# kaist-ina/stellatrain

Hardware: AMD Instinct MI355X
Metric: grad-codec GB/s (dense fp32 in) per GPU; thresholdv16 k=1% on 64 MiB bucket (higher is better)
Workload: dtype f32; 1 GPU; thresholdv16 k=167772 (1%) on 64 MiB fp32 buckets; step = 64 keys (4096 MiB) per GPU in 16 batched calls of 4, call j on stream j % 4; n=16777216, dst_len=167772, streams=4, parallelism=bucket-sharded x1, no collective

## Files before the change

include/stg/codec.h:

```cpp
#ifndef STG_CODEC_H
#define STG_CODEC_H

#include <stddef.h>
#include <stdint.h>

#ifdef __cplusplus
extern "C" {
#endif

#define STG_OK 0
#define STG_ERR_INVALID (-1)
#define STG_ERR_UNKNOWN (-2)
#define STG_ERR_HIP (-3)
#define STG_ERR_UNSUPPORTED (-4)
#define STG_ERR_DEVICE (-5)

typedef struct stg_codec *stg_codec_t;
typedef struct stg_sgd *stg_sgd_t;
typedef struct stg_adam *stg_adam_t;

int stg_codec_create(const char *method, int device, stg_codec_t *out);
int stg_codec_destroy(stg_codec_t h);
const char *stg_codec_name(stg_codec_t h);

// ... 21 lines not shown
int stg_codec_compress_batch_device(stg_codec_t h, const stg_bucket_t *buckets, size_t nbuckets, void *stream);

int stg_merge_compress_batch_device(stg_codec_t h, const stg_bucket_t *buckets, float *const *d_residuals,
                                    size_t nbuckets, void *stream);

int stg_merge_gather_compress_device(stg_codec_t h, const stg_bucket_t *bucket, float *d_residual,
                                     const float *const *d_grads, int num_gpus, void *stream);

int stg_codec_compress_wire_batch_device(stg_codec_t h, const stg_bucket_t *buckets, const int *flags,
                                         size_t nbuckets, void *stream);

typedef struct stg_send_task {
    stg_bucket_t bucket;
    float *d_residual;
    const float *const *d_grads;
    int num_gpus;
    int wire_flag;
} stg_send_task_t;

int stg_merge_send_batch_device(stg_codec_t h, const stg_send_task_t *tasks, size_t ntasks, void *stream);

int stg_codec_get_state(stg_codec_t h, const char *key, const void *key_ptr, float *threshold,
                        float *threshold_inc, void *stream);

int stg_codec_set_timing(stg_codec_t h, int enable);
int stg_codec_get_timing(stg_codec_t h, double *ms3, uint64_t *calls);

int stg_codec_debug_words(stg_codec_t h, void *stream, uint32_t *out, int n);

int stg_debug_tv16_scan_grid(int num_cu, int streams, int hw_queues, uint32_t chunks);

int stg_codec_check(stg_codec_t h);

int stg_scatter_merge_device(const uint32_t *d_idx, const float *d_val, size_t per_rank, int world, size_t n,
                             float *d_dense, uint8_t *d_mark, uint32_t *d_out_idx, float *d_out_val,
                             uint32_t *d_out_count, void *stream);
int stg_scatter_merge_check(void *stream);
int stg_scatter_merge_release(void *stream);

int stg_error_feedback_device(float *d_grad, size_t n, const uint32_t *d_idx, size_t numel, float *d_residual,
                              void *stream);

int stg_sgd_create(int device, float lr, float momentum, float dampening, float weight_decay, int nesterov,
                   int maximize, stg_sgd_t *out);
int stg_sgd_destroy(stg_sgd_t o);
int stg_sgd_optimize_raw_device(stg_sgd_t o, const char *name, float *d_param, uint32_t param_len,
// ... 106 lines not shown
```

stellatrain_amd/csrc/capi.cpp:

```cpp
#include <cmath>
#include <hip/hip_runtime.h>

#include <algorithm>
#include <array>
#include <map>
#include <cstdio>
#include <cstdlib>
#include <cstring>
#include <memory>
#include <mutex>
#include <string>
#include <unordered_map>
#include <vector>

#include <dlfcn.h>

#include "../../include/stg/codec.h"
#include "batch_pack.h"
#include "devbuf.h"
#include "scan_grid.h"
#include "ws.h"

namespace {

// ... 59 lines not shown
    stg::DevBuf<uint32_t> h_idx, h_count;
    uint32_t *pinned_count = nullptr;
    std::mutex wire_mu;
    stg::DevBuf<uint32_t> wst_pos;
    stg::DevBuf<float> wst_val;

    ~Workspace() {
        (void)hipSetDevice(device);
        if (stream) (void)hipStreamSynchronize(stream);
        if (pinned_count) (void)hipHostFree(pinned_count);
    }

    int init() {
        size_t off = 0;
        auto carve = [&](size_t bytes) {
            const size_t o = off;
            off = (off + bytes + 255) & ~size_t(255);
            return o;
        };
        const size_t o_ctl = carve(sizeof(stg::FillCtl));
        const size_t o_cp = carve(sizeof(stg::CallParams));
        const size_t o_rs = carve(sizeof(stg::RSel));
        const size_t o_fail = carve(sizeof(uint32_t));
        const size_t o_cand = carve(sizeof(uint32_t) * stg::CAND_WORDS * stg::MAX_BATCH);
        const size_t o_misc = carve(sizeof(uint32_t) * 64);
        const size_t o_tvt = carve(sizeof(uint64_t));
        const size_t o_wh = carve(sizeof(uint32_t) * 2 * stg::LNBIN);
        const size_t o_larr = carve(sizeof(uint32_t) * stg::LARR_WORDS);
        const size_t o_we = carve(sizeof(uint2) * stg::LNBIN * stg::LBCAP);
        const size_t o_crew = carve(sizeof(stg::CrewCtl) * stg::MAX_BATCH);
        const size_t o_tkc = carve(sizeof(stg::TopkCtl) * 2);
        const size_t o_tkf = carve(sizeof(uint32_t) * 2 * stg::TK2_FINE);
        HIP_TRY(fixed.reserve(off, stream, true));
        char *b = fixed.get();
        d.ctl = reinterpret_cast<stg::FillCtl *>(b + o_ctl);
        d.cp = reinterpret_cast<stg::CallParams *>(b + o_cp);
        d.rsel = reinterpret_cast<stg::RSel *>(b + o_rs);
        d.fail = reinterpret_cast<uint32_t *>(b + o_fail);
        d.cand = reinterpret_cast<uint32_t *>(b + o_cand);
        d.misc = reinterpret_cast<uint32_t *>(b + o_misc);
        d.tv_ticket = reinterpret_cast<uint64_t *>(b + o_tvt);
        d.whist = reinterpret_cast<uint32_t *>(b + o_wh);
        d.larr = reinterpret_cast<uint32_t *>(b + o_larr);
        d.went = reinterpret_cast<uint2 *>(b + o_we);
        d.crew = reinterpret_cast<stg::CrewCtl *>(b + o_crew);
        d.tkctl = reinterpret_cast<stg::TopkCtl *>(b + o_tkc);
        d.tkfine = reinterpret_cast<uint32_t *>(b + o_tkf);
// ... 802 lines not shown
        snprintf(b, sizeof b, "device failure flags 0x%x (details: stg_codec_check)", ws->pinned_count[1]);
        return fail(STG_ERR_DEVICE, b);
    }
    *out_count = *ws->pinned_count;
    return STG_OK;
}

int stg_codec_get_state(stg_codec_t h, const char *key, const void *key_ptr, float *threshold, float *threshold_inc,
                        void *stream) {
    if (!h) return fail(STG_ERR_INVALID, "null codec handle");
    HIP_TRY(hipSetDevice(h->device));
    KeyState *st = nullptr;
    {
        std::lock_guard<std::mutex> g(h->mu);
        auto it = h->slot_of.find(state_key(h->method, key, key_ptr));
        if (it == h->slot_of.end()) return fail(STG_ERR_INVALID, "key has no state yet");
        st = h->slot_ptr(it->second);
    }
    HIP_TRY(hipStreamSynchronize(static_cast<hipStream_t>(stream)));
    KeyState hs;
    HIP_TRY(hipMemcpy(&hs, st, sizeof hs, hipMemcpyDeviceToHost));
    if (threshold) *threshold = hs.t;
    if (threshold_inc) *threshold_inc = hs.inc;
    return STG_OK;
}

int stg_codec_set_timing(stg_codec_t h, int enable) {
    if (!h) return fail(STG_ERR_INVALID, "null codec handle");
    std::lock_guard<std::mutex> g(h->mu);
    h->timing = enable != 0;
    return STG_OK;
}

int stg_codec_get_timing(stg_codec_t h, double *ms3, uint64_t *calls) {
    if (!h || !ms3 || !calls) return fail(STG_ERR_INVALID, "null argument");
    HIP_TRY(hipSetDevice(h->device));
    std::lock_guard<std::mutex> g(h->mu);
    for (auto &e : h->ev_pending) {
        HIP_TRY(hipEventSynchronize(e[2]));
        float a = 0, b = 0, c = 0;
        HIP_TRY(hipEventElapsedTime(&a, e[0], e[1]));
        HIP_TRY(hipEventElapsedTime(&b, e[1], e[2]));
        HIP_TRY(hipEventElapsedTime(&c, e[0], e[2]));
        h->ms_acc[0] += a;
        h->ms_acc[1] += b;
        h->ms_acc[2] += c;
// ... 936 lines not shown
```

stellatrain_amd/csrc/common.h:

```cpp
#pragma once

#include <hip/hip_runtime.h>
#include <stdint.h>

#define STG_WG 256
#define STG_WAVES (STG_WG / 64)

struct KeyState {
    float t;
    float inc;
    uint32_t init;
    uint32_t pad;
};

enum : uint32_t {
    FAIL_SPIN_TIMEOUT = 1u,
    FAIL_CAND_OVERFLOW = 2u,
    FAIL_LEVELS = 4u,
    FAIL_SELECT = 8u,
};

namespace stg {

__device__ __forceinline__ uint32_t f2u(float f) { return __float_as_uint(f); }
__device__ __forceinline__ float u2f(uint32_t u) { return __uint_as_float(u); }

__device__ __forceinline__ uint32_t ford(float f) {
    const uint32_t u = __float_as_uint(f);
    return (u & 0x80000000u) ? ~u : (u | 0x80000000u);
}

template <int CTRL>
__device__ __forceinline__ float dpp_f(float v) {
    return __int_as_float(__builtin_amdgcn_mov_dpp(__float_as_int(v), CTRL, 0xF, 0xF, false));
}
// ... 149 lines not shown
```

stellatrain_amd/csrc/tv16.hip:

```cpp
#include <algorithm>
#include <cstdlib>

#include "scan_grid.h"
#include "tv16_dev.h"

namespace stg {

namespace {

using namespace tv16;
constexpr uint32_t kEfAux = 2;

constexpr uint32_t kTv16Ns = 11;
constexpr uint32_t FWG = (kTv16Ns + 1) * 64;
constexpr uint32_t FNW = FWG / 64;
constexpr uint32_t NS = kTv16Ns;
constexpr uint32_t FIN = NS;
static_assert(NS + 1 <= FNW && FWG <= 1024, "streaming group + finisher fit the workgroup");
constexpr uint32_t kTv16Nbuf = 5;
constexpr uint32_t kTv16ScanD = 3;
constexpr uint32_t NBUF = kTv16Nbuf;
constexpr uint32_t CIDR = 2 * NBUF;
constexpr uint32_t kTv16StageB = 72;
constexpr uint32_t kTv16WlB = 64;
// ... 50 lines not shown
    BucketDesc bk[MAX_BATCH];
    uint32_t nbk;
    uint32_t epoch;
    uint32_t K;
    FillCtl *ctl;
    ChunkDesc *desc;
    uint32_t *cand;
    uint32_t *fail;
    uint32_t *dbg;
};
constexpr uint32_t DBG_DEAD = 1, DBG_DEAD_MAX = 2, DBG_LAUNCHES = 4;
constexpr uint32_t CC_DEAD = 16;

struct Lds {
    float4 stage[NBUF][STAGE_B * 4];
    uint32_t stage_line[NBUF][STAGE_B];
    uint64_t wl[NBUF][WL_B];
    uint32_t nst[NBUF];
    uint32_t nwl[NBUF];
    uint32_t qcnt[NBUF];
    uint32_t wcnt[NBUF];
    uint32_t sdone[NBUF];
    float tval[NBUF], incv[NBUF];
    uint32_t cid[CIDR];
    uint32_t cok[CIDR];
    uint32_t mid[CIDR];
    uint32_t fdone;
    uint4 gb[GB];
};
static_assert(sizeof(Lds) <= TV16_SCAN_LDS, "two scan workgroups and a fill workgroup share a CU");

__device__ __forceinline__ constexpr uint32_t spin_site(uint32_t site) { return FAIL_SPIN_TIMEOUT | (1u << (8 + site)); }

struct Ctx {
    const BatchArgs &A;
    Lds &L;
    uint32_t G, w;
    FillCtl *ctlp;
    uint32_t *candp;
    uint32_t *failp;

    __device__ __forceinline__ uint32_t tag(uint32_t kind) const { return (A.epoch << 8) | kind; }
    __device__ __forceinline__ FillCtl *ctl() const { return ctlp; }
    __device__ __forceinline__ CallCtl *cc() const { return &ctlp->cc[A.epoch & 1u]; }
    __device__ __forceinline__ uint32_t *cand(uint32_t b) const { return candp + (size_t)b * CAND_WORDS; }
    __device__ __forceinline__ void fail(uint32_t bits) const { g_or(failp, bits); }
// ... 3 lines not shown
            st_sc1(failp + 2, w);
            st_sc1(failp + 3, x0);
            st_sc1(failp + 4, x1);
            st_sc1(failp + 5, x2);
            st_sc1(failp + 6, A.epoch);
        }
        uint32_t *rec = failp + 8 + 4 * site;
        if (atomicCAS(rec, 0u, w + 1u) == 0u) {
            st_sc1(rec + 1, x0);
            st_sc1(rec + 2, x1);
            st_sc1(rec + 3, x2);
        }
        for (uint32_t b = 0; b < A.nbk; ++b) st_sc1(A.bk[b].count_out, POISON_COUNT);
    }
    __device__ __forceinline__ uint32_t bucket_of(uint32_t k) const {
        uint32_t b = 0;
        while (b + 1 < A.nbk && k >= A.bk[b + 1].cs) ++b;
        return b;
    }
};

constexpr uint32_t TAG_AGG = 1, TAG_DEC = TV16_TAG_DEC;
constexpr uint32_t DEC_B = TV16_DEC_B, DEC_WIN = TV16_DEC_WIN, DEC_TAIL = TV16_DEC_TAIL;
constexpr uint32_t WIN = TV16_WIN;

template <int STAGE, bool EF, uint32_t SCAN_D>
__device__ __forceinline__ void scan_chunk(Ctx &C, uint32_t j, uint32_t k, uint32_t s) {
    Lds &L = C.L;
    const uint32_t par = j % NBUF;
    if (j >= NBUF) {
        uint64_t st2 = 0;
        uint32_t spins = 0;
        for (; lds_ld(&L.fdone) < j + 1 - NBUF; ++spins) {
            __builtin_amdgcn_s_sleep(2);
            if (spin_expired(spins, st2)) { if (flane() == 0) C.spin_fail(1, j, lds_ld(&L.fdone), s); break; }
        }
    }
    const uint32_t b = C.bucket_of(k);
    const BucketDesc &d = C.A.bk[b];
    const uint32_t c = k - d.cs;
    const uint32_t L0 = c * TV16_CHUNK;
    const uint32_t nl = d.nb > L0 ? std::min(TV16_CHUNK, d.nb - L0) : 0u;
    const float t = uni(d.state->t);
    const uint32_t lane = flane(), q = lane & 3;
    if (s == 0 && lane == 0) { L.tval[par] = t; L.incv[par] = uni(d.state->inc); }
    const uint32_t tb = f2u(t);
    const uint32_t wlo = tb > WIN ? tb - WIN : 0u;
    const uint32_t steps = (nl + 15) / 16;
    const uint32_t mine = steps > s ? (steps - s + NS - 1) / NS : 0u;
    uint32_t cnt_w = 0, win_w = 0;
    const __amdgpu_buffer_rsrc_t rsrc = __builtin_amdgcn_make_buffer_rsrc(
        const_cast<float *>(d.src + (size_t)L0 * 16), 0, nl * 64u, 0x00020000);
    const uint32_t lane_line = s * 16 + (lane >> 2);
    const __amdgpu_buffer_rsrc_t rsrc_r = __builtin_amdgcn_make_buffer_rsrc(
        EF ? d.resid + (size_t)L0 * 16 : nullptr, 0, (EF && d.resid) ? nl * 64u : 0u, 0x00020000);
    auto store_r = [&](uint32_t m, float4 x) {
        uint32_t voff = lane_line * 64u + q * 16u;
        asm volatile("" : "+v"(voff));
        u4v t4;
        t4.x = __float_as_uint(x.x); t4.y = __float_as_uint(x.y); t4.z = __float_as_uint(x.z); t4.w = __float_as_uint(x.w);
        __builtin_amdgcn_raw_buffer_store_b128(t4, rsrc_r, voff + m * (NS * 1024u), 0, kEfAux );
    };
    auto load = [&](uint32_t m) -> float4 {
        uint32_t voff = lane_line * 64u + q * 16u;
        asm volatile("" : "+v"(voff));
        const u4v t4 = __builtin_amdgcn_raw_buffer_load_b128(rsrc, voff + m * (NS * 1024u), 0, 2 );
        return make_float4(__uint_as_float(t4.x), __uint_as_float(t4.y), __uint_as_float(t4.z),
                           __uint_as_float(t4.w));
    };
    float4 v[SCAN_D];
// ... 136 lines not shown
}

template <int STAGE>
__device__ __forceinline__ void finish_chunk(Ctx &C, uint32_t j, uint32_t k) {
    Lds &L = C.L;
    const uint32_t par = j % NBUF;
    const uint32_t lane = flane();
    uint64_t st5 = 0;
    for (uint32_t spins = 0; lds_ld(&L.sdone[par]) < NS; ++spins) {
        __builtin_amdgcn_s_sleep(1);
        if (spin_expired(spins, st5)) { if (lane == 0) C.spin_fail(3, j, lds_ld(&L.sdone[par]), k); break; }
    }
    if (STAGE == 1 || STAGE == 3) {
        release(C, par, j);
        return;
    }
    const uint32_t b = C.bucket_of(k);
    const BucketDesc &d = C.A.bk[b];
    const uint32_t c = k - d.cs;
    const uint32_t L0 = c * TV16_CHUNK;
    const uint32_t nl = d.nb > L0 ? std::min(TV16_CHUNK, d.nb - L0) : 0u;
    const uint32_t qw = uni(L.qcnt[par]);
    const float t = uni(L.tval[par]), inc = uni(L.incv[par]);

    uint32_t P = 0, Wbef = 0;
    if (c) prefix_counts(C, b, c, P, Wbef);
    const uint32_t ww = uni(L.wcnt[par]);

    const uint32_t kb = d.dst_len / 16, r = d.dst_len % 16;
    const uint32_t lim = kb + (r ? 1u : 0u);
    const bool vec = aligned16(d);
    if (P < lim && qw) {
        if (qw <= STAGE_B) {
            const uint32_t q = lane & 3;
            for (uint32_t e0 = 0; e0 < qw; e0 += 16) {
                const uint32_t e = e0 + (lane >> 2);
                if (e >= qw) continue;
                const uint32_t i = L.stage_line[par][e];
                uint32_t g = P;
                for (uint32_t x = 0; x < qw; ++x) g += L.stage_line[par][x] < i;
                if (g >= lim) continue;
                const uint32_t pos = (L0 + i) * 16 + 4 * q;
                const uint32_t len = g == kb ? r : 16u;
                const uint32_t off = 16 * g + 4 * q;
                const float4 x = L.stage[par][e * 4 + q];
                const uint32_t bi = pos + (uint32_t)d.idx_offset;
// ... 19 lines not shown
                    const uint32_t g = base + (uint32_t)__popcll(m & below_mask(lane));
                    if (g < lim) emit_line(d, vec, (L0 + i) * 16, 16 * g, g == kb ? r : 16u);
                }
                base += (uint32_t)__popcll(m);
            }
        }
    }

    if (Wbef + ww + 1 <= CAND_CAP) {
        const uint32_t nwl = uni(lds_ld(&L.nwl[par]));
        uint32_t *cu = C.cand(b);
        uint32_t *cp = cu + CAND_CAP, *ci = cu + 2 * CAND_CAP;
        const uint32_t tb = f2u(t);
        if (nwl <= WL_B && qw <= STAGE_B) {
            static_assert(WL_B == 64, "one listed entry per lane");
            const uint64_t e = lane < nwl ? L.wl[par][lane] : ~0ull;
            const uint32_t mypos = (uint32_t)e;
            const uint32_t li = mypos / 16 - L0;
            uint32_t before = 0, qb = 0;
            for (uint32_t l = 0; l < nwl; ++l) before += (uint32_t)L.wl[par][l] < mypos;
            for (uint32_t x = 0; x < qw; ++x) qb += L.stage_line[par][x] < li;
            if (lane < nwl) {
                const uint32_t idx = Wbef + before;
                st_sc1(&cu[idx], (uint32_t)(e >> 32));
                st_sc1(&cp[idx], mypos);
                st_sc1(&ci[idx], L0 + li - P - qb);
            }
        } else {
            const uint32_t wlo = tb > WIN ? tb - WIN : 0u;
            uint32_t base = Wbef, qb = P;
            for (uint32_t i0 = 0; i0 < nl; i0 += 64) {
                const uint32_t i = i0 + lane;
                const float S = i < nl ? lane_line_sum(d.src + (size_t)(L0 + i) * 16) : 0.f;
                const uint32_t u = f2u(S);
                const bool qf = i < nl && S >= t;
                const bool wf = i < nl && u >= wlo && u < tb;
                const uint64_t mq = __ballot(qf), mw = __ballot(wf);
                if (wf) {
                    const uint32_t idx = base + (uint32_t)__popcll(mw & below_mask(lane));
                    st_sc1(&cu[idx], u);
                    st_sc1(&cp[idx], (L0 + i) * 16);
                    st_sc1(&ci[idx], L0 + i - (qb + (uint32_t)__popcll(mq & below_mask(lane))));
                }
                base += (uint32_t)__popcll(mw);
                qb += (uint32_t)__popcll(mq);
            }
        }
    }
    release(C, par, j);

    if (c + 1 == d.nc) {
        const uint32_t Qtot = P + qw, Wtot = Wbef + ww;
        const uint32_t c0 = Qtot >= lim ? d.dst_len : 16u * Qtot;
        bool tail_cand = false;
        float tail_key = 0.f;
        uint32_t ct = 0;
        if (c0 < d.dst_len && d.tl) {
            const float *tp = d.src + (size_t)d.nb * 16;
            float s = 0.f;
            for (uint32_t i = 0; i < d.tl; ++i) s += tp[i];
            s = uni(s);
            if (s * 16.0f >= t * (float)d.tl) ct = std::min(d.dst_len - c0, d.tl);
            else { tail_cand = true; tail_key = s * 16.0f / (float)d.tl; }
        }
        const uint32_t cnt = c0 + ct;
        const bool regimeB = cnt < d.dst_len;
        if (lane == 0) {
            if (ct) {
                const size_t p0 = (size_t)d.nb * 16;
                for (uint32_t i = 0; i < ct; ++i) {
                    put_pair(d, c0 + i, (uint32_t)(p0 + i) + (uint32_t)d.idx_offset, d.src[p0 + i]);
                }
            }
            d.state->t = regimeB ? (float)((double)t * 0.99) : t + inc;
            d.state->inc = inc;
            d.state->init = 1;
            st_sc1(d.count_out, (uint32_t)std::min<uint64_t>(d.dst_len, (uint64_t)d.nb * 16 + d.tl));
            if (ld_sc1(C.failp)) st_sc1(d.count_out, POISON_COUNT);
        }
        const uint32_t ncand = d.nb - Qtot;
        const uint32_t M = regimeB ? std::min((d.dst_len - cnt + 15u) / 16u, ncand) : 0u;
        uint32_t flags = 0;
        if (regimeB) flags = DEC_B | (tail_cand ? DEC_TAIL : 0u) | (Wtot >= M && Wtot + 1 <= CAND_CAP ? DEC_WIN : 0u);
        Decision &D = C.ctl()->dec[b];
        if (lane == 0) {
            st_sc1(&D.w[1], ((uint64_t)cnt << 32) | M);
            st_sc1(&D.w[2], ((uint64_t)Wtot << 32) | __float_as_uint(tail_key));
            st_sc1(&D.w[3], ((uint64_t)Qtot << 32) | __float_as_uint(t));
        }
        vm_drain();
        if (lane == 0) st_sc1(&D.w[0], ((uint64_t)C.tag(TAG_DEC) << 32) | flags);
    }
}

template <int STAGE, bool EF, bool LONE>
__global__ void __launch_bounds__(1024) __attribute__((amdgpu_waves_per_eu(LONE ? 6 : 8, 8)))
tv16_batch(BatchArgs A) {
    __shared__ Lds L;
    Ctx C{A, L, gridDim.x, blockIdx.x, A.ctl, A.cand, A.fail};
    {
        uint32_t *z = reinterpret_cast<uint32_t *>(&A.ctl->cc[(A.epoch + 1) & 1u]);
        constexpr uint32_t words = sizeof(CallCtl) / 4;
        const uint32_t per = (words + C.G - 1) / C.G;
        const uint32_t z0 = C.w * per, z1 = std::min(words, z0 + per);
        for (uint32_t i = z0 + threadIdx.x; i < z1; i += FWG) st_sc1(z + i, 0u);
    }
// ... 290 lines not shown
```

stellatrain_amd/csrc/tv16fill.hip:

```cpp
#ifndef STG_WIRE_EMIT
#define STG_WIRE_EMIT 0
#endif
#include <algorithm>
#include <cstddef>

#include "tv16_dev.h"

namespace stg {

namespace {

using namespace tv16;

constexpr uint32_t FILL_WG = 512;
constexpr uint32_t FNW_F = FILL_WG / 64;
constexpr uint32_t EMAX = 4096;
constexpr uint32_t VCAP = 6144;
constexpr uint32_t POS_LIM = (1u << 20) - 1;
constexpr uint32_t NONE = 0xffffffffu;
constexpr uint32_t NONE13 = 0x1fffu;
constexpr uint32_t CNONE = 0xffffffu;
constexpr uint32_t NBIN = 1024;
constexpr uint32_t NDEP = 20;
constexpr uint32_t PT = EMAX / FILL_WG;
constexpr uint32_t NJ = VCAP / FILL_WG;
constexpr uint32_t TCAP = 256;
constexpr uint32_t ECAP = 64;
static_assert(VCAP < NONE13, "13-bit node indices");
static_assert(NBIN << 8 == TV16_WIN, "output-sort bins of 256 ulps cover the window");

__device__ __forceinline__ uint32_t dkey_of_pos(uint32_t pos) {
    const uint32_t q = pos + 1, d = depth_of(q);
    return ((q << (19u - d)) << 5) | d;
}
__device__ __forceinline__ uint32_t dk_depth(uint32_t k) { return k & 31u; }
__device__ __forceinline__ uint32_t dk_pos(uint32_t k) { return ((k >> 5) >> (19u - (k & 31u))) - 1u; }
__device__ __forceinline__ uint32_t dk_anc(uint32_t k, uint32_t d) {
    return (((k >> 5) >> (19u - d)) << (19u - d) << 5) | d;
}
__device__ __forceinline__ uint32_t dk_left(uint32_t k) { return (k & ~31u) | (dk_depth(k) + 1); }
__device__ __forceinline__ uint32_t dk_right(uint32_t k) {
    return (((k >> 5) | (1u << (18u - dk_depth(k)))) << 5) | (dk_depth(k) + 1);
}
__device__ __forceinline__ int dk_lca(uint32_t a, uint32_t b) {
    const uint32_t m = min(dk_depth(a), dk_depth(b));
    const uint32_t x = ((a >> 5) ^ (b >> 5)) >> (19u - m);
    return x ? (int)m - (int)(32u - __clz(x)) : (int)m;
}

__device__ __forceinline__ uint32_t r_content(uint2 r) { return r.x & CNONE; }
__device__ __forceinline__ uint32_t r_pos(uint2 r) { return (r.x >> 24) | ((r.y & 0xfffu) << 8); }
__device__ __forceinline__ uint32_t r_right(uint2 r) { return (r.y >> 12) & NONE13; }
// ... 498 lines not shown
            } else {
                for (uint32_t c = 0; c < 4; ++c) {
                    if (4 * q + c < len) {
                        wire_put(oidx, oval, STG_WIRE_EMIT ? wflag : 0u, wend, o + c, bi + c, src[(size_t)pos + 4 * q + c]);
                    }
                }
            }
        }
        return;
    }
    constexpr uint32_t PRE = LONE ? 10 : 8, PREX = PRE;
    constexpr uint32_t KE = LONE ? 10 : 5;
    const uint32_t *cu = d.cand, *cl = d.cand + CAND_CAP, *ci = d.cand + 2 * CAND_CAP;
    uint32_t pk[PRE], pl[PREX], pc[PREX];
#pragma unroll
    for (uint32_t u = 0; u < PRE; ++u) {
        const uint32_t e = tid + u * FILL_WG;
        pk[u] = ld_sc1(&cu[e]);
        if (u < PREX) {
            pl[u] = ld_sc1(&cl[e]);
            pc[u] = ld_sc1(&ci[e]);
        }
    }
    static_assert(PRE * FILL_WG <= CAND_CAP, "prefetch inside the window buffer");
    const uint64_t w0 = ld_sc1(&D.w[0]), w1 = ld_sc1(&D.w[1]), w2 = ld_sc1(&D.w[2]), w3 = ld_sc1(&D.w[3]);
    const uint32_t failed = ld_sc1(A.fail);
    if ((uint32_t)(w0 >> 32) != ((A.epoch << 8) | TV16_TAG_DEC)) {
        if (tid == 0) { g_or(A.fail, FAIL_SPIN_TIMEOUT); st_sc1(d.count_out, POISON_COUNT); }
        return;
    }
    const uint32_t flags = (uint32_t)w0;
    if (!(flags & TV16_DEC_B) || failed) return;
    const uint32_t cnt = (uint32_t)(w1 >> 32), M = (uint32_t)w1;
    const uint32_t Wtot = (uint32_t)(w2 >> 32);
    const float tail_key = u2f((uint32_t)w2);
    const uint32_t Qtot = (uint32_t)(w3 >> 32);
    const float t = u2f((uint32_t)w3);
    const bool tail = (flags & TV16_DEC_TAIL) != 0;
    const uint32_t N = d.nb - Qtot + (tail ? 1u : 0u);
    const uint32_t rem = d.dst_len - cnt;
    if (!M && !tail) return;
    if (A.crew && crew_wants(flags, M, A.mode)) return;
    const uint32_t nhelp = LONE ? A.helpers : 0u;
    CallCtl *const ccp = A.cc;
    const uint32_t tb = f2u(t);
    const uint32_t wlo = tb > TV16_WIN ? tb - TV16_WIN : 0u;
    const bool tail_in = tail && tail_key >= u2f(wlo);
    bool fast = (flags & TV16_DEC_WIN) && N <= POS_LIM && Wtot + (tail_in ? 1u : 0u) > 0 && A.mode != 2u &&
                A.mode != 3u;
    if (!fast && tid == 0) {
        if (!(flags & TV16_DEC_WIN)) atomicAdd(&A.dbg[60], 1u);
        if (N > POS_LIM) atomicAdd(&A.dbg[61], 1u);
    }
    uint32_t *const key = S.u.a.key, *const cix = S.u.a.cix;
    auto kbin = [&](uint32_t kb) -> uint32_t {
        const float k = u2f(kb);
        if (k >= t) return 0u;
        if (!(k > 0.f)) return NBIN - 1;
        return min((tb - 1u - kb) >> 8, NBIN - 1);
    };
    auto okey = [&](uint32_t e) -> uint64_t { return (uint64_t)(~ford(u2f(key[e]))) << 32; };
    auto ksum = [&](uint32_t r) -> float { return u2f(key[S.ord[r]]); };
    uint32_t W = 0, Et = NONE;
    uint32_t *const lines_g = reinterpret_cast<uint32_t *>(d.heap);
    auto line_of = [&](uint32_t i) { return ld_sc1(&lines_g[S.ord[i]]); };
    auto line_lds = [&](uint32_t i) { return S.u.a.line[S.ord[i]]; };
    auto pops = [&](uint32_t &P, uint32_t &tail_rank) {
        for (uint32_t i = tid; i < W; i += FILL_WG)
            if (S.ord[i] == Et) S.flag = i;
        __syncthreads();
        tail_rank = S.flag;
        uint32_t npl = 0;
        for (uint32_t i = tid; i < W; i += FILL_WG) {
            const uint32_t off = 16u * i - (tail_rank < i ? 16u - d.tl : 0u);
            if (off < rem) npl = max(npl, i + 1);
        }
        npl = wave_max(npl);
        if ((tid & 63u) == 0) atomicMax(&S.npop, npl);
        __syncthreads();
        P = S.npop;
    };
    if (tid == 0) { S.flag = NONE; S.nv = 0; S.maxpos = 0; S.npop = 0; S.dmax = 0; S.rn = 0; S.nc = 0; S.nu = 0; S.et = NONE; }
    __syncthreads();
    uint32_t P0 = 0, tail_rank0 = NONE;
    if (fast) {
        SortScratch &X = S.u.a.s;
        stamp(0);
        for (uint32_t i = tid; i < NBIN; i += FILL_WG) X.bin[i] = 0;
        __syncthreads();
#pragma unroll
        for (uint32_t u = 0; u < PRE; ++u)
            if (tid + u * FILL_WG < Wtot) atomicAdd(&X.bin[kbin(pk[u])], 1u);
        for (uint32_t e = tid + PRE * FILL_WG; e < Wtot; e += FILL_WG) atomicAdd(&X.bin[kbin(ld_sc1(&cu[e]))], 1u);
        if (tail_in && tid == 0) atomicAdd(&X.bin[kbin(f2u(tail_key))], 1u);
        __syncthreads();
        stamp(0);
        {
            constexpr uint32_t PER = NBIN / FILL_WG;
            static_assert(PER == 2, "two bins per thread");
            const uint32_t c0 = X.bin[PER * tid], c1 = X.bin[PER * tid + 1], need = M + 2;
            uint32_t tot;
            const uint32_t run = blk_excl_scan<FNW_F>(c0 + c1, S.sh, &tot);
            X.bin[PER * tid] = X.cur[PER * tid] = run;
            X.bin[PER * tid + 1] = X.cur[PER * tid + 1] = run + c0;
            if (run < need && run + c0 >= need) { S.flag = PER * tid + 1; S.nv = run + c0; }
            else if (run + c0 < need && run + c0 + c1 >= need) { S.flag = PER * tid + 2; S.nv = run + c0 + c1; }
            if (tid == 0 && tot < need) { S.flag = NBIN; S.nv = tot; }
            __syncthreads();
        }
        const uint32_t cut = S.flag;
        W = S.nv;
        fast = W <= EMAX;
        if (!fast && tid == 0) atomicAdd(&A.dbg[62], 1u);
        if (fast) {
            auto keep = [&](uint32_t kb, uint32_t line, uint32_t cx, bool is_tail) {
                const uint32_t e = atomicAdd(&X.cur[kbin(kb)], 1u);
                key[e] = kb;
                S.u.a.line[e] = line;
                cix[e] = cx;
                st_sc1(&lines_g[e], line);
                if (is_tail) S.et = e;
            };
#pragma unroll
            for (uint32_t u = 0; u < PRE; ++u) {
                const uint32_t e = tid + u * FILL_WG;
                if (e >= Wtot || kbin(pk[u]) >= cut) continue;
                if (u < PREX) keep(pk[u], pl[u], pc[u], false);
                else keep(pk[u], ld_sc1(&cl[e]), ld_sc1(&ci[e]), false);
            }
            for (uint32_t e = tid + PRE * FILL_WG; e < Wtot; e += FILL_WG) {
                const uint32_t kb = ld_sc1(&cu[e]);
                if (kbin(kb) < cut) keep(kb, ld_sc1(&cl[e]), ld_sc1(&ci[e]), false);
            }
            if (tail_in && tid == 0 && kbin(f2u(tail_key)) < cut) keep(f2u(tail_key), d.nb * 16, N - 1, true);
            __syncthreads();
            stamp(0);
            for (uint32_t e = tid; e < W; e += FILL_WG) {
                const uint32_t bb = kbin(key[e]), lo = X.bin[bb], hi = X.cur[bb];
                const uint64_t k = okey(e) | cix[e];
                uint32_t r = lo;
                for (uint32_t x = lo; x < hi; ++x) r += (okey(x) | cix[x]) < k;
                S.ord[r] = (uint16_t)e;
            }
        }
        Et = S.et;
        __syncthreads();
        if (tid == 0) { S.flag = NONE; S.nv = 0; }
        __syncthreads();
    }
    if (fast) {
        stamp(0);
        pops(P0, tail_rank0);
        uint32_t tie_l = 0;
        for (uint32_t i = tid; i < P0; i += FILL_WG)
            if (i + 1 < W && ksum(i) == ksum(i + 1)) tie_l = 1;
        tie_l = wave_max(tie_l);
        if ((tid & 63u) == 0 && tie_l) S.nv = 1;
        __syncthreads();
        const bool ties = S.nv != 0;
        const uint32_t covered = 16u * W - (Et != NONE ? 16u - d.tl : 0u);
        fast = covered >= rem;
        if (!fast && tid == 0) atomicAdd(&A.dbg[63], 1u);
        if (fast && !ties) {
            emit_all<KE, LONE>(d, cnt, rem, P0, tail_rank0, line_lds, nhelp, ccp, order_g, ready_tag);
            count_path(0);
            stamp(5);
            return;
        }
    }
    if (fast) {
        const uint32_t pc = min(P0, W - 1);
        const float kc = ksum(pc);
        for (uint32_t r = tid; r < W; r += FILL_WG)
            if (ksum(r) == kc && (r + 1 == W || ksum(r + 1) != kc)) S.rn = r + 1;
        __syncthreads();
        fast = S.rn < EMAX;
    }
    if (fast) {
        const uint32_t Rn = S.rn;
        const uint32_t i0 = PT * tid;
        {
            uint32_t stm = 0, nsm = 0;
#pragma unroll
            for (uint32_t u = 0; u < PT; ++u) {
                const uint32_t r = i0 + u;
                if (r < Rn && (r == 0 || ksum(r - 1) != ksum(r))) { stm |= 1u << u; ++nsm; }
            }
            uint32_t tot;
// ... 53 lines not shown
                    }
                }
            }
            if ((__any(bad) || A.mode == 1u) && (tid & 63u) == 0) S.flag2 = 1;
            __syncthreads();
            stamp(0);
            if (!S.flag2) {
                uint16_t *const ord2 = S.u.a.s.tmp;
                for (uint32_t r = tid; r < Rn; r += FILL_WG) {
                    const uint32_t g = S.grp[r], kr = rf_key(cix[S.ord[r]]);
                    uint32_t o = g;
                    for (uint32_t x = g; x < Rn && S.grp[x] == g; ++x) o += rf_key(cix[S.ord[x]]) < kr;
                    ord2[o] = S.ord[r];
                }
                __syncthreads();
                for (uint32_t r = tid; r < Rn; r += FILL_WG) S.ord[r] = ord2[r];
                if (tid == 0) { S.flag = NONE; S.npop = 0; }
                __syncthreads();
                uint32_t P, tail_rank;
                pops(P, tail_rank);
                stamp(0);
                emit_all<KE, LONE>(d, cnt, rem, P, tail_rank, line_lds, nhelp, ccp, order_g, ready_tag);
                count_path(1);
                stamp(0);
                stamp(2);
                return;
            }
        }
        for (uint32_t r = tid; r < Rn; r += FILL_WG) S.u.b.dk[r] = dkey_of_pos(cix[S.ord[r]]);
        __syncthreads();
        counting_sort(S.u.b.s, S.u.b.eo, S.sh, Rn, [&](uint32_t r) { return S.u.b.dk[r] >> 15; },
                      [&](uint32_t r) { return (uint64_t)S.u.b.dk[r]; });
        stamp(0);
        uint32_t kq[PT + 1], rq[PT];
#pragma unroll
        for (uint32_t u = 0; u <= PT; ++u) kq[u] = i0 + u < Rn ? S.u.b.dk[S.u.b.eo[i0 + u]] : 0u;
#pragma unroll
        for (uint32_t u = 0; u < PT; ++u) rq[u] = i0 + u < Rn ? S.u.b.eo[i0 + u] : 0u;
        const uint32_t kp = (i0 >= 1 && i0 - 1 < Rn) ? S.u.b.dk[S.u.b.eo[i0 - 1]] : 0u;
        auto Lof = [&](uint32_t u) -> int {
            const uint32_t i = i0 + u;
            return (i >= 1 && i < Rn) ? dk_lca(u ? kq[u - 1] : kp, kq[u]) : -1;
        };
        uint32_t nmine = 0;
#pragma unroll
        for (uint32_t u = 0; u < PT; ++u) {
// ... 162 lines not shown
            nc = wave_sum(nc);
            if ((tid & 63u) == 0) { atomicMax(&S.maxpos, mp); atomicAdd(&S.nc, nc); }
            __syncthreads();
            fast = S.nc == Rn;
        }
        if (fast) {
            for (uint32_t r = tid; r < Rn; r += FILL_WG) {
                const uint32_t g = S.grp[r], kr = rf_key(S.u.f.fpos[r]);
                uint32_t o = g;
                for (uint32_t x = g; x < Rn && S.grp[x] == g; ++x) o += rf_key(S.u.f.fpos[x]) < kr;
                S.u.f.ord2[o] = S.ord[r];
            }
            __syncthreads();
            for (uint32_t r = tid; r < Rn; r += FILL_WG) S.ord[r] = S.u.f.ord2[r];
            if (tid == 0) { S.flag = NONE; S.npop = 0; }
            __syncthreads();
            uint32_t P, tail_rank;
            pops(P, tail_rank);
            stamp(0);
            if (STG_FILL_STAMPS && tid == 0 && b == 0) A.dbg[45] = P;
            if (S.maxpos + P < N && P <= Rn) {
                emit_all<KE, LONE>(d, cnt, rem, P, tail_rank, line_of, nhelp, ccp, order_g, ready_tag);
                count_path(2);
                stamp(1);
                return;
            }
            fast = false;
        }
    }
    __syncthreads();
    if ((flags & TV16_DEC_WIN) && A.mode != 2u) {
        const uint32_t P0 = (rem + 15u) / 16u, seln = min(P0 + 1u, N - 1u);
        if (Wtot >= seln + 1u || Wtot + (tail ? 1u : 0u) == N) {
            WideLds &Wl = *reinterpret_cast<WideLds *>(fill_lds);
            LeadIn I;
            I.lk = cu;
            I.lp = cl;
            I.lc = ci;
            I.n = Wtot;
            I.tail = tail ? 1u : 0u;
            I.tail_bits = f2u(tail_key);
            I.N = N;
            I.nb = d.nb;
            I.rem = rem;
            I.tl = d.tl;
            I.g = reinterpret_cast<uint32_t *>(d.heap);
            I.dbg = A.dbg;
            I.lvl1 = NONE;
            I.r1 = 0;
            I.gcap = 2u * (d.nb + 64u);
            I.positions = true;
            const LeadOut O = leader(Wl, I);
            if (O.ok) {
                const uint32_t *const opos = O.ordpos;
                emit_all<KE, LONE>(d, cnt, rem, O.P, O.tail_rank, [&](uint32_t i) { return ld_sc1(&opos[i]); }, nhelp,
                                   ccp, order_g, ready_tag);
                if (tid == 0) atomicAdd(&A.dbg[52], 1u);
                return;
            }
            if (tid == 0) atomicAdd(&A.dbg[54], 1u);
            __syncthreads();
        }
    }
    if (tid == 0) { S.flag = NONE; S.npop = 0; }
    __syncthreads();
    stamp(3);
    count_path(3);
    if (LONE && A.helpers && tid == 0) {
        st_sc1(&A.cc->pad[2], 0u);
        __builtin_amdgcn_s_waitcnt(0);
        st_sc1(&A.cc->pad[1], ready_tag);
    }
    full_path(S, d, cnt, N, t, tail, tail_key, A.fail);
    stamp(0);
}

}

constexpr size_t LFIN_LDS = std::max(std::max(sizeof(FillLds), sizeof(LfinLds)), sizeof(WideLdsBig));
static_assert(LFIN_LDS <= 160 * 1024, "one lfin workgroup per CU");
// ... 23 lines not shown
```

stellatrain_amd/csrc/ws.h:

```cpp
#pragma once

#include <hip/hip_runtime.h>
#include <stdint.h>

#include "common.h"

namespace stg {

constexpr uint32_t CAND_CAP = 8192;
constexpr uint32_t CAND_WORDS = 4 * CAND_CAP;
constexpr uint32_t TV16_WIN = 1u << 18;
constexpr uint32_t TV16_SCAN_LDS = 35584;

constexpr uint32_t TV_TILE = 8192;
constexpr uint32_t TOPK_SUP_CAP = 1024;
constexpr uint32_t TOPK_LIST_CAP = 4096;
constexpr uint32_t TOPK_LIST_TILES = 8192;
constexpr uint32_t TV_MAXG = 2048;
constexpr uint32_t TV_SCAP = 4096;

constexpr uint32_t RS_BINS = 2048;
constexpr uint32_t RS_SHARDS = 8;
constexpr uint32_t RS_SH_HIST = 4;

constexpr uint32_t MAX_BATCH = 32;
constexpr uint32_t TV16_CHUNK = 2048;
struct CallCtl {
    uint32_t next;
    uint32_t pad[31];
    uint32_t crew_ticket[32];
    uint32_t crew_done[32];
};
struct alignas(32) Decision {
    uint64_t w[4];
};
constexpr uint32_t TV16_DEC_B = 1, TV16_DEC_WIN = 2, TV16_DEC_TAIL = 4;
constexpr uint32_t TV16_TAG_DEC = 3;
constexpr uint32_t POISON_COUNT = 0xffffffffu;
struct FillCtl {
    CallCtl cc[2];
    Decision dec[MAX_BATCH];
};
struct alignas(16) ChunkDesc {
    uint64_t agg;
    uint64_t pad;
};

struct CallParams {
    float t;
    float inc;
    uint32_t pad[2];
};

struct RSel {
    uint32_t prefix;
    uint32_t mask;
    uint32_t rank;
    uint32_t cnt_gt;
    uint32_t done;
// ... 460 lines not shown
```

Baseline: 6189 GB/s.

## Adapt tv16 candidate window width per key and double candidate capacity

Replaces the fixed threshold-window width with a per-key adaptive width stored in the codec state. The width grows when the candidate list misses or overflows and shrinks after a run of calm calls. Candidate list capacity is doubled, writes beyond it are bounds-checked, and the fill's histogram bins scale with the window width. The aim is to keep more calls on the fast windowed fill path instead of falling back to the full path. The cost is a larger scratch carve, extra per-call state updates, and a deep-selection guard that can force some calls onto the slow path.

Result: no change. 6188 GB/s (-0.0%).

```diff
diff --git a/include/stg/codec.h b/include/stg/codec.h
--- a/include/stg/codec.h
+++ b/include/stg/codec.h
@@ -67,6 +67,8 @@
 
 int stg_codec_get_state(stg_codec_t h, const char *key, const void *key_ptr, float *threshold,
                         float *threshold_inc, void *stream);
+
+int stg_codec_get_window(stg_codec_t h, const char *key, uint32_t *width, uint32_t *calm, void *stream);
 
 int stg_codec_set_timing(stg_codec_t h, int enable);
 int stg_codec_get_timing(stg_codec_t h, double *ms3, uint64_t *calls);
diff --git a/stellatrain_amd/csrc/capi.cpp b/stellatrain_amd/csrc/capi.cpp
--- a/stellatrain_amd/csrc/capi.cpp
+++ b/stellatrain_amd/csrc/capi.cpp
@@ -105,7 +105,9 @@
         const size_t o_cp = carve(sizeof(stg::CallParams));
         const size_t o_rs = carve(sizeof(stg::RSel));
         const size_t o_fail = carve(sizeof(uint32_t));
-        const size_t o_cand = carve(sizeof(uint32_t) * stg::CAND_WORDS * stg::MAX_BATCH);
+        static_assert(stg::tv16win::cand_carve_words() >= (uint64_t)stg::CAND_WORDS * stg::MAX_BATCH,
+                      "the carve covers the lists of a full launch");
+        const size_t o_cand = carve(sizeof(uint32_t) * (size_t)stg::tv16win::cand_carve_words());
         const size_t o_misc = carve(sizeof(uint32_t) * 64);
         const size_t o_tvt = carve(sizeof(uint64_t));
         const size_t o_wh = carve(sizeof(uint32_t) * 2 * stg::LNBIN);
@@ -954,6 +956,24 @@
     HIP_TRY(hipMemcpy(&hs, st, sizeof hs, hipMemcpyDeviceToHost));
     if (threshold) *threshold = hs.t;
     if (threshold_inc) *threshold_inc = hs.inc;
+    return STG_OK;
+}
+
+int stg_codec_get_window(stg_codec_t h, const char *key, uint32_t *width, uint32_t *calm, void *stream) {
+    if (!h) return fail(STG_ERR_INVALID, "null codec handle");
+    HIP_TRY(hipSetDevice(h->device));
+    KeyState *st = nullptr;
+    {
+        std::lock_guard<std::mutex> g(h->mu);
+        auto it = h->slot_of.find(state_key(h->method, key, nullptr));
+        if (it == h->slot_of.end()) return fail(STG_ERR_INVALID, "key has no state yet");
+        st = h->slot_ptr(it->second);
+    }
+    HIP_TRY(hipStreamSynchronize(static_cast<hipStream_t>(stream)));
+    KeyState hs;
+    HIP_TRY(hipMemcpy(&hs, st, sizeof hs, hipMemcpyDeviceToHost));
+    if (width) *width = stg::tv16win::win_c(hs.win);
+    if (calm) *calm = stg::tv16win::win_calm(hs.win);
     return STG_OK;
 }
 
diff --git a/stellatrain_amd/csrc/common.h b/stellatrain_amd/csrc/common.h
--- a/stellatrain_amd/csrc/common.h
+++ b/stellatrain_amd/csrc/common.h
@@ -10,7 +10,7 @@
     float t;
     float inc;
     uint32_t init;
-    uint32_t pad;
+    uint32_t win;
 };
 
 enum : uint32_t {
diff --git a/stellatrain_amd/csrc/tv16.hip b/stellatrain_amd/csrc/tv16.hip
--- a/stellatrain_amd/csrc/tv16.hip
+++ b/stellatrain_amd/csrc/tv16.hip
@@ -96,6 +96,7 @@
     uint32_t wcnt[NBUF];
     uint32_t sdone[NBUF];
     float tval[NBUF], incv[NBUF];
+    uint32_t cwin[NBUF];
     uint32_t cid[CIDR];
     uint32_t cok[CIDR];
     uint32_t mid[CIDR];
@@ -145,7 +146,6 @@
 
 constexpr uint32_t TAG_AGG = 1, TAG_DEC = TV16_TAG_DEC;
 constexpr uint32_t DEC_B = TV16_DEC_B, DEC_WIN = TV16_DEC_WIN, DEC_TAIL = TV16_DEC_TAIL;
-constexpr uint32_t WIN = TV16_WIN;
 
 template <int STAGE, bool EF, uint32_t SCAN_D>
 __device__ __forceinline__ void scan_chunk(Ctx &C, uint32_t j, uint32_t k, uint32_t s) {
@@ -166,9 +166,10 @@
     const uint32_t nl = d.nb > L0 ? std::min(TV16_CHUNK, d.nb - L0) : 0u;
     const float t = uni(d.state->t);
     const uint32_t lane = flane(), q = lane & 3;
-    if (s == 0 && lane == 0) { L.tval[par] = t; L.incv[par] = uni(d.state->inc); }
+    const uint32_t cw = uni(d.state->win);
+    if (s == 0 && lane == 0) { L.tval[par] = t; L.incv[par] = uni(d.state->inc); L.cwin[par] = cw; }
     const uint32_t tb = f2u(t);
-    const uint32_t wlo = tb > WIN ? tb - WIN : 0u;
+    const uint32_t wlo = tv16win::win_lo(tb, tv16win::win_c(cw));
     const uint32_t steps = (nl + 15) / 16;
     const uint32_t mine = steps > s ? (steps - s + NS - 1) / NS : 0u;
     uint32_t cnt_w = 0, win_w = 0;
@@ -351,6 +352,7 @@
     const uint32_t nl = d.nb > L0 ? std::min(TV16_CHUNK, d.nb - L0) : 0u;
     const uint32_t qw = uni(L.qcnt[par]);
     const float t = uni(L.tval[par]), inc = uni(L.incv[par]);
+    const uint32_t cw = uni(L.cwin[par]), wc = tv16win::win_c(cw);
 
     uint32_t P = 0, Wbef = 0;
     if (c) prefix_counts(C, b, c, P, Wbef);
@@ -416,12 +418,16 @@
             for (uint32_t x = 0; x < qw; ++x) qb += L.stage_line[par][x] < li;
             if (lane < nwl) {
                 const uint32_t idx = Wbef + before;
-                st_sc1(&cu[idx], (uint32_t)(e >> 32));
-                st_sc1(&cp[idx], mypos);
-                st_sc1(&ci[idx], L0 + li - P - qb);
+                if (idx < CAND_CAP) {
+                    st_sc1(&cu[idx], (uint32_t)(e >> 32));
+                    st_sc1(&cp[idx], mypos);
+                    st_sc1(&ci[idx], L0 + li - P - qb);
+                } else {
+                    C.fail(FAIL_CAND_OVERFLOW);
+                }
             }
         } else {
-            const uint32_t wlo = tb > WIN ? tb - WIN : 0u;
+            const uint32_t wlo = tv16win::win_lo(tb, wc);
             uint32_t base = Wbef, qb = P;
             for (uint32_t i0 = 0; i0 < nl; i0 += 64) {
                 const uint32_t i = i0 + lane;
@@ -432,9 +438,13 @@
                 const uint64_t mq = __ballot(qf), mw = __ballot(wf);
                 if (wf) {
                     const uint32_t idx = base + (uint32_t)__popcll(mw & below_mask(lane));
-                    st_sc1(&cu[idx], u);
-                    st_sc1(&cp[idx], (L0 + i) * 16);
-                    st_sc1(&ci[idx], L0 + i - (qb + (uint32_t)__popcll(mq & below_mask(lane))));
+                    if (idx < CAND_CAP) {
+                        st_sc1(&cu[idx], u);
+                        st_sc1(&cp[idx], (L0 + i) * 16);
+                        st_sc1(&ci[idx], L0 + i - (qb + (uint32_t)__popcll(mq & below_mask(lane))));
+                    } else {
+                        C.fail(FAIL_CAND_OVERFLOW);
+                    }
                 }
                 base += (uint32_t)__popcll(mw);
                 qb += (uint32_t)__popcll(mq);
@@ -459,6 +469,8 @@
         }
         const uint32_t cnt = c0 + ct;
         const bool regimeB = cnt < d.dst_len;
+        const uint32_t ncand = d.nb - Qtot;
+        const uint32_t M = regimeB ? std::min((d.dst_len - cnt + 15u) / 16u, ncand) : 0u;
         if (lane == 0) {
             if (ct) {
                 const size_t p0 = (size_t)d.nb * 16;
@@ -469,13 +481,13 @@
             d.state->t = regimeB ? (float)((double)t * 0.99) : t + inc;
             d.state->inc = inc;
             d.state->init = 1;
+            d.state->win = tv16win::win_next(cw, regimeB, M, Wtot);
             st_sc1(d.count_out, (uint32_t)std::min<uint64_t>(d.dst_len, (uint64_t)d.nb * 16 + d.tl));
             if (ld_sc1(C.failp)) st_sc1(d.count_out, POISON_COUNT);
         }
-        const uint32_t ncand = d.nb - Qtot;
-        const uint32_t M = regimeB ? std::min((d.dst_len - cnt + 15u) / 16u, ncand) : 0u;
-        uint32_t flags = 0;
-        if (regimeB) flags = DEC_B | (tail_cand ? DEC_TAIL : 0u) | (Wtot >= M && Wtot + 1 <= CAND_CAP ? DEC_WIN : 0u);
+        uint32_t flags = wc << TV16_DEC_CSHIFT;
+        const bool holds = (Wtot >= M + 2u || Wtot == ncand) && Wtot >= M && tv16win::list_fits(Wtot);
+        if (regimeB) flags |= DEC_B | (tail_cand ? DEC_TAIL : 0u) | (holds ? DEC_WIN : 0u);
         Decision &D = C.ctl()->dec[b];
         if (lane == 0) {
             st_sc1(&D.w[1], ((uint64_t)cnt << 32) | M);
diff --git a/stellatrain_amd/csrc/tv16_window.h b/stellatrain_amd/csrc/tv16_window.h
--- /dev/null
+++ b/stellatrain_amd/csrc/tv16_window.h
@@ -0,0 +1,76 @@
+#pragma once
+
+#include <stdint.h>
+
+#if defined(__HIPCC__) || defined(__CUDACC__)
+#define TV16W_HD __host__ __device__
+#else
+#define TV16W_HD
+#endif
+
+namespace stg {
+namespace tv16win {
+
+constexpr uint32_t UNIT_LOG2 = 16;
+constexpr uint32_t C_BASE = 4;
+constexpr uint32_t C_MAX = 9;
+constexpr uint32_t CALM_CALLS = 32;
+constexpr uint32_t C_MASK = 0xffu, CALM_SHIFT = 8, CALM_MASK = 0xffu;
+static_assert(C_MAX <= C_MASK && CALM_CALLS <= CALM_MASK, "both fields fit their byte");
+static_assert(C_BASE >= 1 && C_BASE <= C_MAX, "the range is not empty");
+
+TV16W_HD constexpr uint32_t win_c(uint32_t word) {
+    return (word & C_MASK) < C_BASE ? C_BASE : (word & C_MASK) > C_MAX ? C_MAX : (word & C_MASK);
+}
+TV16W_HD constexpr uint32_t win_calm(uint32_t word) { return (word >> CALM_SHIFT) & CALM_MASK; }
+TV16W_HD constexpr uint32_t win_word(uint32_t c, uint32_t calm) { return (calm << CALM_SHIFT) | c; }
+TV16W_HD constexpr uint32_t win_ulps(uint32_t c) { return c << UNIT_LOG2; }
+TV16W_HD constexpr uint32_t win_lo(uint32_t tb, uint32_t c) { return tb > win_ulps(c) ? tb - win_ulps(c) : 0u; }
+
+constexpr uint32_t NBIN = 1024;
+constexpr uint32_t BIN_LOG2 = 8;
+static_assert((NBIN << BIN_LOG2) == win_ulps(C_BASE), "at the base width the bins are 256 ulps, as the one-bucket path's");
+TV16W_HD constexpr uint32_t bin_shift(uint32_t c) {
+    uint32_t s = 0;
+    while (((NBIN << BIN_LOG2) << s) < win_ulps(c)) ++s;
+    return s;
+}
+TV16W_HD constexpr uint32_t win_bin(uint32_t tb, uint32_t kb, uint32_t c) {
+    return (tb - 1u - kb) >> (BIN_LOG2 + bin_shift(c));
+}
+static_assert(bin_shift(C_BASE) == 0 && ((NBIN << BIN_LOG2) << bin_shift(C_MAX)) >= win_ulps(C_MAX), "bins cover the window");
+
+constexpr uint32_t MAX_BATCH = 32;
+constexpr uint32_t CAND_CAP = 16384;
+constexpr uint32_t CAND_ARRAYS = 4;
+constexpr uint32_t CAND_WORDS = CAND_ARRAYS * CAND_CAP;
+constexpr uint32_t ORDER_ARRAY = 3;
+constexpr uint32_t EMAX = 4096;
+constexpr uint32_t FILL_WG = 512;
+constexpr uint32_t FILL_PRE_MAX = 10;
+TV16W_HD constexpr bool list_fits(uint32_t Wtot) { return Wtot + 1u <= CAND_CAP; }
+TV16W_HD constexpr uint64_t cand_carve_words() { return (uint64_t)CAND_WORDS * MAX_BATCH; }
+static_assert(EMAX + 1 <= CAND_CAP, "what the fill orders from LDS is a part of the list");
+static_assert(FILL_PRE_MAX * FILL_WG <= CAND_CAP, "the fill's prefetch stays inside one list array");
+static_assert((ORDER_ARRAY + 1) * CAND_CAP <= CAND_WORDS, "the order (<= CAND_CAP pops) has an array of its own");
+
+TV16W_HD constexpr bool win_miss(bool regimeB, uint32_t M, uint32_t Wtot) {
+    return regimeB && (Wtot < M + 2u || !list_fits(Wtot));
+}
+TV16W_HD constexpr bool win_calm_call(bool regimeB, uint32_t M, uint32_t Wtot, uint32_t c) {
+    return !regimeB || (!win_miss(regimeB, M, Wtot) && (uint64_t)4u * Wtot * (c - 1u) >= (uint64_t)5u * (M + 2u) * c);
+}
+TV16W_HD constexpr uint32_t win_next(uint32_t word, bool regimeB, uint32_t M, uint32_t Wtot) {
+    const uint32_t c = win_c(word);
+    if (win_miss(regimeB, M, Wtot)) {
+        const uint32_t step = c / 2u > 2u ? c / 2u : 2u;
+        return win_word(c + step > C_MAX ? C_MAX : c + step, 0u);
+    }
+    if (!win_calm_call(regimeB, M, Wtot, c)) return win_word(c, 0u);
+    const uint32_t calm = win_calm(word) + 1u;
+    if (calm < CALM_CALLS) return win_word(c, calm);
+    return win_word(c > C_BASE ? c - 1u : C_BASE, 0u);
+}
+
+}
+}
diff --git a/stellatrain_amd/csrc/tv16fill.hip b/stellatrain_amd/csrc/tv16fill.hip
--- a/stellatrain_amd/csrc/tv16fill.hip
+++ b/stellatrain_amd/csrc/tv16fill.hip
@@ -12,22 +12,22 @@
 
 using namespace tv16;
 
-constexpr uint32_t FILL_WG = 512;
+constexpr uint32_t FILL_WG = tv16win::FILL_WG;
 constexpr uint32_t FNW_F = FILL_WG / 64;
-constexpr uint32_t EMAX = 4096;
+constexpr uint32_t EMAX = tv16win::EMAX;
 constexpr uint32_t VCAP = 6144;
 constexpr uint32_t POS_LIM = (1u << 20) - 1;
 constexpr uint32_t NONE = 0xffffffffu;
 constexpr uint32_t NONE13 = 0x1fffu;
 constexpr uint32_t CNONE = 0xffffffu;
-constexpr uint32_t NBIN = 1024;
+constexpr uint32_t NBIN = tv16win::NBIN;
 constexpr uint32_t NDEP = 20;
 constexpr uint32_t PT = EMAX / FILL_WG;
 constexpr uint32_t NJ = VCAP / FILL_WG;
 constexpr uint32_t TCAP = 256;
 constexpr uint32_t ECAP = 64;
 static_assert(VCAP < NONE13, "13-bit node indices");
-static_assert(NBIN << 8 == TV16_WIN, "output-sort bins of 256 ulps cover the window");
+static_assert(NBIN << 8 == TV16_WIN, "output-sort bins of 256 ulps cover the base window (wider: tv16_window.h bin_shift)");
 
 __device__ __forceinline__ uint32_t dkey_of_pos(uint32_t pos) {
     const uint32_t q = pos + 1, d = depth_of(q);
@@ -572,7 +572,7 @@
             pc[u] = ld_sc1(&ci[e]);
         }
     }
-    static_assert(PRE * FILL_WG <= CAND_CAP, "prefetch inside the window buffer");
+    static_assert(PRE <= tv16win::FILL_PRE_MAX && PRE * FILL_WG <= CAND_CAP, "prefetch inside the window buffer");
     const uint64_t w0 = ld_sc1(&D.w[0]), w1 = ld_sc1(&D.w[1]), w2 = ld_sc1(&D.w[2]), w3 = ld_sc1(&D.w[3]);
     const uint32_t failed = ld_sc1(A.fail);
     if ((uint32_t)(w0 >> 32) != ((A.epoch << 8) | TV16_TAG_DEC)) {
@@ -594,20 +594,26 @@
     const uint32_t nhelp = LONE ? A.helpers : 0u;
     CallCtl *const ccp = A.cc;
     const uint32_t tb = f2u(t);
-    const uint32_t wlo = tb > TV16_WIN ? tb - TV16_WIN : 0u;
+    const uint32_t wc = tv16win::win_c(flags >> TV16_DEC_CSHIFT);
+    const uint32_t wlo = tv16win::win_lo(tb, wc), bsh = tv16win::BIN_LOG2 + tv16win::bin_shift(wc);
     const bool tail_in = tail && tail_key >= u2f(wlo);
+    const bool deep = M + 2u > EMAX;
     bool fast = (flags & TV16_DEC_WIN) && N <= POS_LIM && Wtot + (tail_in ? 1u : 0u) > 0 && A.mode != 2u &&
-                A.mode != 3u;
+                A.mode != 3u && !deep;
     if (!fast && tid == 0) {
         if (!(flags & TV16_DEC_WIN)) atomicAdd(&A.dbg[60], 1u);
         if (N > POS_LIM) atomicAdd(&A.dbg[61], 1u);
+        if (deep && (flags & TV16_DEC_WIN) && N <= POS_LIM && A.mode != 2u && A.mode != 3u) atomicAdd(&A.dbg[62], 1u);
     }
     uint32_t *const key = S.u.a.key, *const cix = S.u.a.cix;
     auto kbin = [&](uint32_t kb) -> uint32_t {
         const float k = u2f(kb);
         if (k >= t) return 0u;
         if (!(k > 0.f)) return NBIN - 1;
-        return min((tb - 1u - kb) >> 8, NBIN - 1);
+        return min((tb - 1u - kb) >> bsh, NBIN - 1);
+    };
+    auto count_wide = [&]() {
+        if (tid == 0 && wc > tv16win::C_BASE) atomicAdd(&A.dbg[30], 1u);
     };
     auto okey = [&](uint32_t e) -> uint64_t { return (uint64_t)(~ford(u2f(key[e]))) << 32; };
     auto ksum = [&](uint32_t r) -> float { return u2f(key[S.ord[r]]); };
@@ -641,7 +647,10 @@
 #pragma unroll
         for (uint32_t u = 0; u < PRE; ++u)
             if (tid + u * FILL_WG < Wtot) atomicAdd(&X.bin[kbin(pk[u])], 1u);
-        for (uint32_t e = tid + PRE * FILL_WG; e < Wtot; e += FILL_WG) atomicAdd(&X.bin[kbin(ld_sc1(&cu[e]))], 1u);
+        constexpr uint32_t PF = PRE * FILL_WG;
+        const uint32_t nrest = Wtot > PF ? Wtot - PF : 0u;
+        each_b<uint32_t, 4>(nrest, [&](uint32_t i) { return ld_sc1(&cu[PF + i]); },
+                            [&](uint32_t, uint32_t kb) { atomicAdd(&X.bin[kbin(kb)], 1u); });
         if (tail_in && tid == 0) atomicAdd(&X.bin[kbin(f2u(tail_key))], 1u);
         __syncthreads();
         stamp(0);
@@ -678,10 +687,8 @@
                 if (u < PREX) keep(pk[u], pl[u], pc[u], false);
                 else keep(pk[u], ld_sc1(&cl[e]), ld_sc1(&ci[e]), false);
             }
-            for (uint32_t e = tid + PRE * FILL_WG; e < Wtot; e += FILL_WG) {
-                const uint32_t kb = ld_sc1(&cu[e]);
-                if (kbin(kb) < cut) keep(kb, ld_sc1(&cl[e]), ld_sc1(&ci[e]), false);
-            }
+            each_b<uint3, 4>(nrest, [&](uint32_t i) { return make_uint3(ld_sc1(&cu[PF + i]), ld_sc1(&cl[PF + i]), ld_sc1(&ci[PF + i])); },
+                             [&](uint32_t, uint3 x) { if (kbin(x.x) < cut) keep(x.x, x.y, x.z, false); });
             if (tail_in && tid == 0 && kbin(f2u(tail_key)) < cut) keep(f2u(tail_key), d.nb * 16, N - 1, true);
             __syncthreads();
             stamp(0);
@@ -714,6 +721,7 @@
         if (fast && !ties) {
             emit_all<KE, LONE>(d, cnt, rem, P0, tail_rank0, line_lds, nhelp, ccp, order_g, ready_tag);
             count_path(0);
+            count_wide();
             stamp(5);
             return;
         }
@@ -813,6 +821,7 @@
                 stamp(0);
                 emit_all<KE, LONE>(d, cnt, rem, P, tail_rank, line_lds, nhelp, ccp, order_g, ready_tag);
                 count_path(1);
+                count_wide();
                 stamp(0);
                 stamp(2);
                 return;
@@ -1021,6 +1030,7 @@
             if (S.maxpos + P < N && P <= Rn) {
                 emit_all<KE, LONE>(d, cnt, rem, P, tail_rank, line_of, nhelp, ccp, order_g, ready_tag);
                 count_path(2);
+                count_wide();
                 stamp(1);
                 return;
             }
@@ -1055,6 +1065,7 @@
                 emit_all<KE, LONE>(d, cnt, rem, O.P, O.tail_rank, [&](uint32_t i) { return ld_sc1(&opos[i]); }, nhelp,
                                    ccp, order_g, ready_tag);
                 if (tid == 0) atomicAdd(&A.dbg[52], 1u);
+                count_wide();
                 return;
             }
             if (tid == 0) atomicAdd(&A.dbg[54], 1u);
diff --git a/stellatrain_amd/csrc/ws.h b/stellatrain_amd/csrc/ws.h
--- a/stellatrain_amd/csrc/ws.h
+++ b/stellatrain_amd/csrc/ws.h
@@ -4,12 +4,14 @@
 #include <stdint.h>
 
 #include "common.h"
+#include "tv16_window.h"
 
 namespace stg {
 
-constexpr uint32_t CAND_CAP = 8192;
-constexpr uint32_t CAND_WORDS = 4 * CAND_CAP;
-constexpr uint32_t TV16_WIN = 1u << 18;
+constexpr uint32_t CAND_CAP = tv16win::CAND_CAP;
+constexpr uint32_t CAND_WORDS = tv16win::CAND_WORDS;
+constexpr uint32_t TV16_WIN = tv16win::win_ulps(tv16win::C_BASE);
+static_assert(TV16_WIN == 1u << 18, "the one-bucket path's 1,024 bins of 256 ulps");
 constexpr uint32_t TV16_SCAN_LDS = 35584;
 
 constexpr uint32_t TV_TILE = 8192;
@@ -23,7 +25,7 @@
 constexpr uint32_t RS_SHARDS = 8;
 constexpr uint32_t RS_SH_HIST = 4;
 
-constexpr uint32_t MAX_BATCH = 32;
+constexpr uint32_t MAX_BATCH = tv16win::MAX_BATCH;
 constexpr uint32_t TV16_CHUNK = 2048;
 struct CallCtl {
     uint32_t next;
@@ -35,6 +37,7 @@
     uint64_t w[4];
 };
 constexpr uint32_t TV16_DEC_B = 1, TV16_DEC_WIN = 2, TV16_DEC_TAIL = 4;
+constexpr uint32_t TV16_DEC_CSHIFT = 8;
 constexpr uint32_t TV16_TAG_DEC = 3;
 constexpr uint32_t POISON_COUNT = 0xffffffffu;
 struct FillCtl {
```
